# marksho-sfdc/TransmogrifAI

Measured on AMD Instinct MI355X. Metric: end-to-end AutoML wall-clock + hold-out AuPR, 10M-row binary-class tabular, lower is better.
Workload: dtype fp32; 1 GPU; binary-10m; model=BinaryClassificationModelSelector(default grid), rows=10000000, raw_columns=200, cv_folds=3, global_batch=10000000, max_training_sample=1000000, parallelism=single

## Files before the change

transmogrifai_amd/ops/csrc/hip/tree_hist_kernels.hip:

```cpp
#include <hip/hip_runtime.h>
#include <algorithm>
#include <cstdlib>
#include <stdint.h>
#include <math.h>

#include "common/tree_rules.hpp"
#include "hip/tmog_hip_abi.h"
#include "hip/tree_dev.hpp"

namespace {

using namespace tmog;

template <int MODE>
__device__ __forceinline__ int4 stage_row(uint32_t e, int64_t model, int64_t stride, const float* __restrict__ y,
                                          const float* __restrict__ t1, const float* __restrict__ t2,
                                          const float* __restrict__ qs, int wide) {
  const int64_t r = ent_row(e, wide);
  const float w = (float)ent_w(e, wide);
  int4 s;
  s.x = (int)e;
  if (MODE == 0) {
    s.y = (int)ent_w(e, wide); s.z = (int)y[r]; s.w = 0;
  } else if (MODE == 1) {
    const float t = t1[model * stride + r];
    const float wt = w * t;
    s.y = (int)ent_w(e, wide);
    s.z = (int)rintf(wt * qs[1]);
    s.w = (int)rintf((wt * t) * qs[2]);
  } else {
    s.y = (int)rintf((w * t1[model * stride + r]) * qs[0]);
    s.z = (int)rintf((w * t2[model * stride + r]) * qs[1]);
    s.w = 0;
  }
  return s;
}

template <int MODE>
__device__ __forceinline__ void add_row(int* my, int bin, int S, int s0, int Sc, const int4& st) {
  if (MODE == 0) {
    const int c = st.z - s0;
    if (c >= 0 && c < Sc) atomicAdd(my + bin * Sc + c, st.y);
  } else if (MODE == 1) {
    int* hb = my + bin * Sc;
    const int v[3] = {st.y, st.z, st.w};
    for (int k = 0; k < Sc; ++k) atomicAdd(hb + k, v[s0 + k]);
  } else {
    int* hb = my + bin * Sc;
    if (Sc == 2) {
      atomicAdd(hb, st.y); atomicAdd(hb + 1, st.z);
    } else {
      atomicAdd(hb, s0 ? st.z : st.y);
    }
  }
}

constexpr int kCsrU = 16;
constexpr int kCsrG = 8;

template <bool MAX>
__device__ __forceinline__ int wave_reduce32(int v) {
#define TM_DPP_STEP(CTRL, ROWS)                                                         \
  {                                                                                     \
    const int t = __builtin_amdgcn_update_dpp(0, v, CTRL, ROWS, 0xF, false);           \
    v = MAX ? max(v, t) : v + t;                                                        \
  }
  TM_DPP_STEP(0x111, 0xF) TM_DPP_STEP(0x112, 0xF) TM_DPP_STEP(0x114, 0xF) TM_DPP_STEP(0x118, 0xF)
  TM_DPP_STEP(0x142, 0xA) TM_DPP_STEP(0x143, 0xC)
#undef TM_DPP_STEP
  return __builtin_amdgcn_readlane(v, 63);
}

__device__ __forceinline__ void hist_csr_item(const HistItem& it, const uint32_t* __restrict__ rows,
                                              const int32_t* __restrict__ node_model,
                                              const int64_t* __restrict__ node_hist_off, int64_t* __restrict__ hist,
                                              int B, int S, const float* __restrict__ t1,
                                              const float* __restrict__ t2, int64_t stride,
                                              const float* __restrict__ qscale, int skip_bin,
                                              const int64_t* __restrict__ csr_ptr,
                                              const uint16_t* __restrict__ csr_col, int* lds,
                                              const int2* __restrict__ gh, int wide) {
  const int nf = it.nf;
  int* a0 = lds;
  int* a1 = lds + nf;
  const int lane = threadIdx.x & 63;
  const int wave = threadIdx.x >> 6;
  const int nwaves = blockDim.x >> 6;
  const int soff = (2 * nf + 3) & ~3;
  int4* stg = reinterpret_cast<int4*>(lds + soff) + wave * 64;
  int* lens = lds + soff + 4 * 64 * nwaves + wave * 64;
  for (int i = threadIdx.x; i < 2 * nf; i += blockDim.x) lds[i] = 0;
  __syncthreads();
  const int64_t model = node_model ? node_model[it.node] : 0;
  const float* qs = qscale + model * S;
  const uint32_t* rp = rows + it.begin;
  const int64_t cnt = it.count;
  const float* t1m = t1 + model * stride;
  const float* t2m = t2 + model * stride;
  const int64_t step = (int64_t)nwaves * 64;
  const int2* ghp = gh ? gh + it.begin : nullptr;
  uint32_t e_n = 0;
  float g_n = 0.f, h_n = 0.f;
  int2 q_n = make_int2(0, 0);
  int64_t p0_n = 0, p1_n = 0;
  if ((int64_t)wave * 64 < cnt) {
    const int64_t i0 = min((int64_t)wave * 64 + lane, cnt - 1);
    e_n = rp[i0];
    const int64_t r = ent_row(e_n, wide);
    if (ghp) q_n = ghp[i0];
    else { g_n = t1m[r]; h_n = t2m[r]; }
    p0_n = csr_ptr[r]; p1_n = csr_ptr[r + 1];
  }
  for (int64_t base = (int64_t)wave * 64; base < cnt; base += step) {
    const int nrows = (int)min((int64_t)64, cnt - base);
    const float wt = (float)ent_w(e_n, wide);
    int4 mine;
    mine.x = (int)e_n;
    mine.y = ghp ? q_n.x : (int)rintf((wt * g_n) * qs[0]);
    mine.z = ghp ? q_n.y : (int)rintf((wt * h_n) * qs[1]);
    mine.w = 0;
    const int64_t q0 = p0_n;
    const int len = lane < nrows ? (int)(p1_n - p0_n) : 0;
    const bool more = base + step < cnt;
    const int64_t i_n = min(base + step + lane, cnt - 1);
    if (more) e_n = rp[i_n];
    stg[lane] = make_int4(mine.y, mine.z, (int)(uint32_t)(uint64_t)q0, (int)((uint64_t)q0 >> 32));
    lens[lane] = len;
    const int mx = wave_reduce32<true>(len);
    const int W = mx <= 8 ? 8 : mx <= 16 ? 16 : mx <= 32 ? 32 : 64;
    const int RPI = 64 / W;
    const int rs = lane / W, k = lane - rs * W;
    __builtin_amdgcn_s_waitcnt(0xC07F);
    __builtin_amdgcn_wave_barrier();
    for (int j0 = 0; j0 < nrows; j0 += RPI * kCsrG) {
      int col[kCsrG];
      bool ok[kCsrG];
#pragma unroll
      for (int u = 0; u < kCsrG; ++u) {
        const int src = j0 + u * RPI + rs;
        const int sl = min(src, 63);
        const int ln = src < nrows ? lens[sl] : 0;
        const int4 rr = stg[sl];
        const int64_t k0 = (int64_t)(((uint64_t)(uint32_t)rr.w << 32) | (uint64_t)(uint32_t)rr.z);
        ok[u] = k < ln;
        col[u] = csr_col[ok[u] ? k0 + k : k0 > 0 ? k0 - 1 : 0];
      }
      __builtin_amdgcn_sched_barrier(0);
      if (j0 == 0 && more) {
        const int64_t r = ent_row(e_n, wide);
        if (ghp) q_n = ghp[i_n];
        else { g_n = t1m[r]; h_n = t2m[r]; }
        p0_n = csr_ptr[r]; p1_n = csr_ptr[r + 1];
      }
      __builtin_amdgcn_sched_barrier(0);
#pragma unroll
      for (int u = 0; u < kCsrG; ++u)
        if (ok[u]) {
          const int2 gh = *reinterpret_cast<const int2*>(&stg[min(j0 + u * RPI + rs, 63)]);
          atomicAdd(a0 + col[u], gh.x);
          atomicAdd(a1 + col[u], gh.y);
        }
      if (W == 64) {
#pragma unroll
        for (int u = 0; u < kCsrG; ++u) {
          const int src = j0 + u * RPI + rs;
          const int sl = min(src, 63);
          const int ln = src < nrows ? lens[sl] : 0;
          if (ln <= 64) continue;
          const int4 rr = stg[sl];
          const int64_t k0 = (int64_t)(((uint64_t)(uint32_t)rr.w << 32) | (uint64_t)(uint32_t)rr.z);
          for (int kk = k + 64; kk < ln; kk += 64) {
            const int c = csr_col[k0 + kk];
            atomicAdd(a0 + c, rr.x);
            atomicAdd(a1 + c, rr.y);
          }
        }
      }
    }
    __builtin_amdgcn_wave_barrier();
  }
  __syncthreads();
  int64_t* out = hist + node_hist_off[it.node] + (int64_t)it.fg0 * B * S;
  const int per = B * S;
  const bool excl = (it.excl & TMOG_ITEM_SOLE) != 0;
  for (int k = threadIdx.x; k < nf * S; k += blockDim.x) {
    const int f = k / S, s = k - f * S;
    const int v = s ? a1[f] : a0[f];
    int64_t* w = out + (int64_t)f * per + s;
    if (excl) *w = v;
    else if (v != 0) atomicAdd(reinterpret_cast<unsigned long long*>(w), (unsigned long long)(int64_t)v);
  }
}


constexpr int kWideU = 16;

__device__ __forceinline__ void hist_wide_item(const HistItem& it, const uint8_t* __restrict__ Xb, int F, int col0,
                                               const uint32_t* __restrict__ rows,
                                               const int32_t* __restrict__ node_model,
                                               const int64_t* __restrict__ node_hist_off, int64_t* __restrict__ hist,
                                               int B, const float* __restrict__ t1, const float* __restrict__ t2,
                                               int64_t stride, const float* __restrict__ qscale, int skip_bin,
                                               int* lds, const int2* __restrict__ gh, int wide) {
  const int FG = it.nf;
  const int ND = (FG + 3) >> 2;
  const int NP = ND <= 1 ? 1 : ND <= 2 ? 2 : ND <= 4 ? 4 : ND <= 8 ? 8 : 16;
  const int RPI = 64 / NP;
  const int lane = threadIdx.x & 63, wave = threadIdx.x >> 6, nwaves = blockDim.x >> 6;
  const int rs = lane / NP, d = lane - rs * NP;
  const int pos = lane & 15;
  const int sub = (B + 1) * 16;
  unsigned long long* tab = reinterpret_cast<unsigned long long*>(lds);
  const int twords = 4 * sub;
  const int toff = (2 * twords + 3) & ~3;
  int4* stage = reinterpret_cast<int4*>(lds + toff) + wave * 64;
  int* tot = lds + toff + 4 * 64 * nwaves;
  for (int i = threadIdx.x; i < twords; i += blockDim.x) tab[i] = 0ull;
  if (threadIdx.x < 2) tot[threadIdx.x] = 0;
  __syncthreads();
  const bool sparse = skip_bin >= 0;
  const int64_t model = node_model ? node_model[it.node] : 0;
  const float* qs = qscale + model * 2;
  const uint32_t* rp = rows + it.begin;
  const int64_t cnt = it.count;
  const uint64_t xbase = (uint64_t)(uintptr_t)(Xb + col0);
  const uint32_t xlo = __builtin_amdgcn_readfirstlane((uint32_t)xbase);
  const uint32_t xhi = __builtin_amdgcn_readfirstlane((uint32_t)(xbase >> 32));
  const __amdgpu_buffer_rsrc_t xrs = __builtin_amdgcn_make_buffer_rsrc(
      (void*)(uintptr_t)(((uint64_t)xhi << 32) | xlo), (short)0, 0x7FFFFFFF, 0x00020000);
  const uint32_t lane_off = 4u * (uint32_t)min(d, ND - 1);
  const float* t1m = t1 + model * stride;
  const float* t2m = t2 + model * stride;
  const int64_t step = (int64_t)nwaves * 64;
  const int2* ghp = gh ? gh + it.begin : nullptr;
  uint32_t e_n = 0;
  float g_n = 0.f, h_n = 0.f;
  int2 q_n = make_int2(0, 0);
  if ((int64_t)wave * 64 < cnt) {
    const int64_t i0 = min((int64_t)wave * 64 + lane, cnt - 1);
    e_n = rp[i0];
    if (ghp) q_n = ghp[i0];
    else {
      g_n = t1m[ent_row(e_n, wide)];
      h_n = t2m[ent_row(e_n, wide)];
    }
  }
  for (int64_t base = (int64_t)wave * 64; base < cnt; base += step) {
    const int nrows = (int)min((int64_t)64, cnt - base);
    const float wt = (float)ent_w(e_n, wide);
    int4 mine;
    mine.x = (int)e_n;
    mine.y = ghp ? q_n.x : (int)rintf((wt * g_n) * qs[0]);
    mine.z = ghp ? q_n.y : (int)rintf((wt * h_n) * qs[1]);
    mine.w = 0;
    const bool more = base + step < cnt;
    const int64_t i_n = min(base + step + lane, cnt - 1);
    if (more) {
      e_n = rp[i_n];
      if (ghp) q_n = ghp[i_n];
    }
    stage[lane] = make_int4(mine.y, mine.z, mine.x, 0);
    if (sparse) {
      const int a = wave_reduce32<false>(lane < nrows ? mine.y : 0);
      const int b = wave_reduce32<false>(lane < nrows ? mine.z : 0);
      if (lane == 0) {
        atomicAdd(tot, a);
        atomicAdd(tot + 1, b);
      }
    }
    __builtin_amdgcn_s_waitcnt(0xC07F);
    __builtin_amdgcn_wave_barrier();
    {
      uint32_t off[kWideU], w[kWideU];
#pragma unroll
      for (int u = 0; u < kWideU; ++u)
        off[u] = (wide ? (uint32_t)stage[min(u * RPI + rs, 63)].z * (uint32_t)F
                       : __umul24((uint32_t)stage[min(u * RPI + rs, 63)].z & 0xFFFFFFu, (uint32_t)F)) + lane_off;
#pragma unroll
      for (int u = 0; u < kWideU; ++u) w[u] = __builtin_amdgcn_raw_buffer_load_b32(xrs, (int)off[u], 0, 0);
      __builtin_amdgcn_sched_barrier(0);
      if (more && !ghp) {
        g_n = t1m[ent_row(e_n, wide)];
        h_n = t2m[ent_row(e_n, wide)];
      }
      __builtin_amdgcn_sched_barrier(0);
#pragma unroll
      for (int u = 0; u < kWideU; ++u) {
        const bool live = u * RPI + rs < nrows;
        const int2 st = *reinterpret_cast<const int2*>(&stage[min(u * RPI + rs, 63)]);
        const unsigned long long pk = live ? ((unsigned long long)(uint32_t)st.x << 32) + (unsigned long long)(uint32_t)st.y
                                           : 0ull;
#pragma unroll
        for (int k = 0; k < 4; ++k) {
          const int bin = (int)((w[u] >> (8 * k)) & 0xFFu);
          atomicAdd(tab + k * sub + bin * 16 + pos, 4 * d + k < FG ? pk : 0ull);
        }
      }
    }
    __builtin_amdgcn_wave_barrier();
  }
  __syncthreads();
  if (NP < 16) {
    for (int i = threadIdx.x; i < 4 * B * NP; i += blockDim.x) {
      const int r = i / NP, dd = i - r * NP;
      unsigned long long* row = tab + (r / B) * sub + (r % B) * 16;
      unsigned long long acc = row[dd];
      for (int c = NP; c < 16; c += NP) acc += row[c + dd];
      row[dd] = acc;
    }
    __syncthreads();
  }
  auto tix = [sub](int f, int b) { return (f & 3) * sub + b * 16 + (f >> 2); };
  if (sparse) {
    for (int f = threadIdx.x; f < FG; f += blockDim.x) {
      long long g = 0, h = 0;
      for (int b = 0; b < B; ++b) {
        if (b == skip_bin) continue;
        const unsigned long long v = tab[tix(f, b)];
        g += (long long)v >> 32;
        h += (long long)(v & 0xFFFFFFFFull);
      }
      const long long mg = (long long)tot[0] - g, mh = (long long)tot[1] - h;
      tab[tix(f, B)] = ((unsigned long long)mg << 32) + (unsigned long long)(uint32_t)mh;
    }
    __syncthreads();
  }
  int64_t* out = hist + node_hist_off[it.node] + (int64_t)it.fg0 * B * 2;
  const bool excl = (it.excl & TMOG_ITEM_SOLE) != 0;
  for (int k = threadIdx.x; k < FG * B; k += blockDim.x) {
    const int f = k / B, b = k - f * B;
    const unsigned long long v = tab[tix(f, (sparse && b == skip_bin) ? B : b)];
    const int64_t g = (long long)v >> 32, h = (long long)(v & 0xFFFFFFFFull);
    int64_t* o = out + (int64_t)k * 2;
    if (excl) {
      o[0] = g;
      o[1] = h;
    } else {
      if (g != 0) atomicAdd(reinterpret_cast<unsigned long long*>(o), (unsigned long long)g);
      if (h != 0) atomicAdd(reinterpret_cast<unsigned long long*>(o + 1), (unsigned long long)h);
    }
  }
}

constexpr int HIST_U = 16;

__device__ int g_hist_debug = 0;

template <int OCC>
__global__ void __launch_bounds__(256) __attribute__((amdgpu_waves_per_eu(OCC))) hist_wide_kernel(
    const uint8_t* __restrict__ Xb, int F, const uint32_t* __restrict__ rows, const HistItem* __restrict__ items,
    const int32_t* __restrict__ node_feat_off, const int32_t* __restrict__ feat_list,
    const int32_t* __restrict__ node_model, const int64_t* __restrict__ node_hist_off, int64_t* __restrict__ hist,
    int B, const float* __restrict__ t1, const float* __restrict__ t2, int64_t stride,
    const float* __restrict__ qscale, int skip_bin, const int2* __restrict__ gh, int wide,
    const uint8_t* __restrict__ Xh, int Fh) {
  extern __shared__ int lds_w[];
  if (g_hist_debug & 2) return;
  const HistItem it = items[blockIdx.x];
  hist_wide_item(it, Xh, Fh, feat_list[node_feat_off[it.node] + it.fg0], rows, node_model, node_hist_off, hist, B,
                 t1, t2, stride, qscale, skip_bin, lds_w, gh, wide);
}


template <int MODE, bool GEN = true>
__global__ void __launch_bounds__(256) hist_build_kernel(
    const uint8_t* __restrict__ Xb, int F, const uint32_t* __restrict__ rows, const HistItem* __restrict__ items,
    const int32_t* __restrict__ node_feat_off, const int32_t* __restrict__ feat_list,
    const int32_t* __restrict__ node_model, const int64_t* __restrict__ node_hist_off, int64_t* __restrict__ hist,
    int B, int S, const float* __restrict__ y, const float* __restrict__ t1, const float* __restrict__ t2,
    int64_t stride, const float* __restrict__ qscale, int skip_bin, const int64_t* __restrict__ csr_ptr,
    const uint16_t* __restrict__ csr_col, int Sc, const int2* __restrict__ gh, const int* __restrict__ dcount,
    int wide, const uint8_t* __restrict__ Xh, int Fh) {
  extern __shared__ __attribute__((aligned(16))) int lds[];
  if (dcount != nullptr && (int)blockIdx.x >= *dcount) return;
  const HistItem it = items[blockIdx.x];
  const int s0 = ((it.excl >> TMOG_ITEM_SC_SHIFT) & 0xFF) * Sc;
  const int sc = min(Sc, S - s0);
  if (MODE == 2 && g_hist_debug) {
    if ((g_hist_debug & 1) && (it.excl & TMOG_ITEM_CSR)) return;
    if ((g_hist_debug & 2) && !(it.excl & TMOG_ITEM_CSR)) return;
  }
  if (MODE == 2 && (it.excl & TMOG_ITEM_CSR)) {
    hist_csr_item(it, rows, node_model, node_hist_off, hist, B, S, t1, t2, stride, qscale, skip_bin, csr_ptr,
                  csr_col, lds, gh, wide);
    return;
  }
  if (MODE == 2 && (it.excl & TMOG_ITEM_WIDE)) {
    hist_wide_item(it, Xh, Fh, feat_list[node_feat_off[it.node] + it.fg0], rows, node_model, node_hist_off, hist, B,
                   t1, t2, stride, qscale, skip_bin, lds, gh, wide);
    return;
  }
  if constexpr (!GEN) {
    return;
  } else {
  const int FG = it.nf;
  const int R = 64 / FG;
  const int rowstride = B * sc + 1;
  const int ncopy_words = R * FG * rowstride;
  const int lane = threadIdx.x & 63;
  const int wave = threadIdx.x >> 6;
  const int nwaves = blockDim.x >> 6;
  int4* stage = reinterpret_cast<int4*>(lds + ((ncopy_words + 3) & ~3)) + wave * 64;
  int* tot = lds + ((ncopy_words + 3) & ~3) + 4 * 64 * 4;
  const bool sparse = MODE == 2 && skip_bin >= 0;
  const bool regacc = sparse && (it.excl & TMOG_ITEM_REG);
  const bool excl = (it.excl & TMOG_ITEM_SOLE) != 0;
  for (int i = threadIdx.x; i < ncopy_words; i += blockDim.x) lds[i] = 0;
  if (threadIdx.x < TM_MAX_S) tot[threadIdx.x] = 0;
  __syncthreads();

  const int rsub = lane / FG;
  const int fidx = lane - rsub * FG;
  const bool active = rsub < R;
  const int feat = active ? feat_list[node_feat_off[it.node] + it.fg0 + fidx] : 0;
  const int64_t model = node_model ? node_model[it.node] : 0;
  const float* qs = qscale + model * S;
  int* my = lds + (rsub * FG + fidx) * rowstride;
  const uint32_t* rp = rows + it.begin;
  const int64_t cnt = it.count;

  int racc0 = 0, racc1 = 0;
  for (int64_t base = (int64_t)wave * 64; base < cnt; base += (int64_t)nwaves * 64) {
    const int64_t ri = min(base + lane, cnt - 1);
    const int nrows = (int)min((int64_t)64, cnt - base);
    int4 mine;
    if (MODE == 2 && gh) {
      const int2 q = gh[it.begin + ri];
      mine = make_int4((int)rp[ri], q.x, q.y, 0);
    } else {
      mine = stage_row<MODE>(rp[ri], model, stride, y, t1, t2, qs, wide);
    }
    stage[lane] = mine;
    if (sparse) {
      const int a = wave_reduce32<false>(lane < nrows ? mine.y : 0);
      const int b = wave_reduce32<false>(lane < nrows ? mine.z : 0);
      if (lane == 0) {
        atomicAdd(tot, a);
        atomicAdd(tot + 1, b);
      }
    }
    __builtin_amdgcn_s_waitcnt(0xC07F);
    __builtin_amdgcn_wave_barrier();
    if (regacc) {
      for (int j0 = 0; j0 < nrows; j0 += R * 8) {
        int4 st[8];
        int bin[8];
#pragma unroll
        for (int u = 0; u < 8; ++u) st[u] = stage[min(j0 + u * R + rsub, 63)];
#pragma unroll
        for (int u = 0; u < 8; ++u) bin[u] = (int)Xb[(int64_t)ent_row((uint32_t)st[u].x, wide) * F + feat];
#pragma unroll
        for (int u = 0; u < 8; ++u) {
          const bool hit = j0 + u * R + rsub < nrows && bin[u] == 0;
          racc0 += hit ? st[u].y : 0;
          racc1 += hit ? st[u].z : 0;
        }
      }
      __builtin_amdgcn_wave_barrier();
      continue;
    }
    for (int j0 = 0; j0 < nrows; j0 += R * HIST_U) {
      int4 st[HIST_U];
      int bin[HIST_U];
#pragma unroll
      for (int u = 0; u < HIST_U; ++u) st[u] = stage[min(j0 + u * R + rsub, 63)];
#pragma unroll
      for (int u = 0; u < HIST_U; ++u) bin[u] = (int)Xb[(int64_t)ent_row((uint32_t)st[u].x, wide) * F + feat];
#pragma unroll
      for (int u = 0; u < HIST_U; ++u)
        if (active && j0 + u * R + rsub < nrows && bin[u] != skip_bin) add_row<MODE>(my, bin[u], S, s0, sc, st[u]);
    }
    __builtin_amdgcn_wave_barrier();
  }
  __syncthreads();

  int64_t* out = hist + node_hist_off[it.node] + (int64_t)it.fg0 * B * S;
  const int words = FG * B * S;
  if (regacc) {
    if (active) {
      atomicAdd(my, racc0);
      atomicAdd(my + 1, racc1);
    }
    __syncthreads();
  }
  if (sparse) {
    if (R > 1) {
      for (int k = threadIdx.x; k < words; k += blockDim.x) {
        const int f = k / (B * S);
        const int rem = k - f * (B * S);
        int acc = 0;
        for (int r = 0; r < R; ++r) acc += lds[(r * FG + f) * rowstride + rem];
        lds[f * rowstride + rem] = acc;
      }
      __syncthreads();
    }
    for (int t = threadIdx.x; t < FG * S; t += blockDim.x) {
      const int f = t / S, s = t - (t / S) * S;
      int* row = lds + f * rowstride;
      int sum = 0;
      for (int b = 0; b < B; ++b) sum += (b == skip_bin) ? 0 : row[b * S + s];
      row[skip_bin * S + s] = tot[s] - sum;
    }
    __syncthreads();
    const int wlimit = (it.excl & TMOG_ITEM_LIVE0) ? S : B * S;
    for (int k = threadIdx.x; k < words; k += blockDim.x) {
      const int f = k / (B * S);
      if (k - f * (B * S) >= wlimit) continue;
      const int64_t acc = lds[f * rowstride + (k - f * (B * S))];
      if (excl) out[k] = acc;
      else if (acc != 0) atomicAdd(reinterpret_cast<unsigned long long*>(out + k), (unsigned long long)acc);
    }
    return;
  }
  const int cwords = FG * B * sc;
  for (int k = threadIdx.x; k < cwords; k += blockDim.x) {
    const int f = k / (B * sc);
    const int rem = k - f * (B * sc);
    int64_t acc = 0;
    for (int r = 0; r < R; ++r) acc += lds[(r * FG + f) * rowstride + rem];
    const int bin = rem / sc, c = rem - bin * sc;
    int64_t* w = out + ((int64_t)f * B + bin) * S + s0 + c;
    if (excl) *w = acc;
    else if (acc != 0) atomicAdd(reinterpret_cast<unsigned long long*>(w), (unsigned long long)acc);
  }
  }
}

__device__ __forceinline__ int live_word(int k, int dense, int per, int S) {
  if (dense < 0 || k < dense) return k;
  const int t = k - dense, f = t / S;
  return dense + f * per + (t - f * S);
}

__global__ void hist_subtract_kernel(int64_t* __restrict__ hist, const int64_t* __restrict__ parent,
                                     const int64_t* __restrict__ parent_off, const int64_t* __restrict__ small_off,
                                     const int64_t* __restrict__ out_off, const int64_t* __restrict__ size, int n,
                                     int64_t dense, int per, int S) {
  const int j = blockIdx.y;
  if (j >= n) return;
  const int sz = (int)live_words(size[j], dense, per, S);
  const int dn = (int)dense;
  const int64_t* p = parent + parent_off[j];
  const int64_t* s = hist + small_off[j];
  int64_t* o = hist + out_off[j];
  for (int k = blockIdx.x * blockDim.x + threadIdx.x; k < sz; k += gridDim.x * blockDim.x) {
    const int w = live_word(k, dn, per, S);
    o[w] = p[w] - s[w];
  }
}

__global__ void zero_segments_kernel(int64_t* __restrict__ hist, const int64_t* __restrict__ off,
                                     const int64_t* __restrict__ size, int n, int64_t dense, int per, int S,
                                     int n_dense, const int* __restrict__ dcnt) {
  const int j = blockIdx.y;
  if (dcnt != nullptr) {
    n = dcnt[0];
    n_dense = dcnt[1];
  }
  if (j >= n) return;
  int64_t* o = hist + off[j];
  const int64_t dj = j < n_dense ? dense : 0;
  const int sz = (int)live_words(size[j], dj, per, S);
  const int dn = (int)dj;
  for (int k = blockIdx.x * blockDim.x + threadIdx.x; k < sz; k += gridDim.x * blockDim.x)
    o[live_word(k, dn, per, S)] = 0;
}

inline size_t hist_lds_bytes(int B, int Sc) {
  return (size_t)(((64 * (B * Sc + 1)) + 3) & ~3) * sizeof(int) + 4 * 64 * sizeof(int4) + TM_MAX_S * sizeof(int);
}
inline size_t hist_wide_lds_bytes(int B) {
  return (size_t)((2 * (64 * (B + 1) + 17) + 3) & ~3) * sizeof(int) + 4 * 64 * sizeof(int4) + 4 * sizeof(int);
}

}

int tmog::prime_tree_hist() { return prime_kernel(&zero_segments_kernel); }

extern "C" {

int tmog_hip_debug_flags(int flags) {
  return (int)hipMemcpyToSymbol(HIP_SYMBOL(g_hist_debug), &flags, sizeof(int));
}

int tmog_hip_hist_build(const uint8_t* Xb, int F, const uint32_t* rows, const void* items, int n_items,
                        const int32_t* node_feat_off, const int32_t* feat_list, const int32_t* node_model,
                        const int64_t* node_hist_off, int64_t* hist, int B, int mode, int S, const float* y,
                        const float* t1, const float* t2, int64_t stride, const float* qscale, int skip_bin,
                        const int64_t* csr_ptr, const uint16_t* csr_col, int Sc, int n_wide, int need_general,
                        hipStream_t stream, const int32_t* gh_words, const int* dcount, int wide_rows,
                        const uint8_t* Xh, int Fh) {
  if (n_items == 0) return 0;
  if (Xh == nullptr) {
    Xh = Xb;
    Fh = F;
  }
  if (dcount != nullptr && n_wide != 0) return -2;
  const int2* gh = reinterpret_cast<const int2*>(gh_words);
  if (gh && mode != 2) return -2;
  if (Sc <= 0 || Sc > S) Sc = S;
  size_t lds = hist_lds_bytes(B, Sc);
  if (mode == 2 && S == 2) lds = std::max(lds, hist_wide_lds_bytes(B));
  if (lds > 160 * 1024) return -2;
  if (skip_bin >= B || (mode == 2 && skip_bin >= 0 && (S != 2 || Sc != S))) return -2;
  if (mode == 0 && S > TM_WIDE_MAX_S) return -2;
  if ((csr_ptr != nullptr) != (csr_col != nullptr) || (csr_ptr && (mode != 2 || skip_bin <= 0))) return -2;
  const HistItem* it = (const HistItem*)items;
  if (n_wide < 0 || n_wide > n_items || (n_wide > 0 && (mode != 2 || S != 2))) return -2;
  static const bool split_wide = [] { const char* e = std::getenv("TMOG_HIST_WIDE_SPLIT"); return e && e[0] == '1'; }();
  if (!split_wide) n_wide = 0;
  if (n_wide > 0) {
    static const int occ = [] { const char* e = std::getenv("TMOG_HIST_WIDE_OCC"); return e ? std::atoi(e) : 6; }();
#define TM_HIST_WIDE(OCC)                                                                                      \
  hipLaunchKernelGGL(hist_wide_kernel<OCC>, dim3(n_wide), dim3(256), lds, stream, Xb, F, rows, it, node_feat_off, \
                     feat_list, node_model, node_hist_off, hist, B, t1, t2, stride, qscale, skip_bin, gh, wide_rows, Xh, Fh)
    if (occ >= 7) TM_HIST_WIDE(7);
    else TM_HIST_WIDE(6);
#undef TM_HIST_WIDE
    it += n_wide;
    n_items -= n_wide;
    if (n_items == 0) return (int)hipGetLastError();
  }
  const int skip = (mode == 0 || mode == 1) ? -1 : skip_bin;
#define TM_HIST(...)                                                                                           \
  hipLaunchKernelGGL((hist_build_kernel<__VA_ARGS__>), dim3(n_items), dim3(256), lds, stream, Xb, F, rows, it, \
                     node_feat_off, feat_list, node_model, node_hist_off, hist, B, S, y, t1, t2, stride, qscale, \
                     skip, csr_ptr, csr_col, Sc, gh, dcount, wide_rows, Xh, Fh)
  if (mode == 0) TM_HIST(0);
  else if (mode == 1) TM_HIST(1);
  else if (need_general) TM_HIST(2);
  else TM_HIST(2, false);
#undef TM_HIST
  return (int)hipGetLastError();
}

int tmog_hip_hist_subtract(int64_t* hist, const int64_t* parent, const int64_t* parent_off, const int64_t* small_off,
                           const int64_t* out_off, const int64_t* size, int n, int64_t max_size, int64_t dense,
                           int per, int S, hipStream_t stream) {
  if (n == 0) return 0;
  if (max_size >= (int64_t)1 << 31) return -2;
  int gx = (int)min((live_words(max_size, dense, per, S) + 255) / 256, (int64_t)1024);
  if (gx < 1) gx = 1;
  hipLaunchKernelGGL(hist_subtract_kernel, dim3(gx, n), dim3(256), 0, stream, hist, parent, parent_off, small_off,
                     out_off, size, n, dense, per, S);
  return (int)hipGetLastError();
}

int tmog_hip_zero_segments(int64_t* hist, const int64_t* off, const int64_t* size, int n, int64_t max_size,
                           int64_t dense, int per, int S, hipStream_t stream, int n_dense, const int* dn) {
  if (n == 0) return 0;
  if (max_size >= (int64_t)1 << 31) return -2;
  const int64_t lw = std::max(live_words(max_size, dense, per, S), live_words(max_size, 0, per, S));
  int gx = (int)min((lw + 255) / 256, (int64_t)1024);
  if (gx < 1) gx = 1;
  hipLaunchKernelGGL(zero_segments_kernel, dim3(gx, n), dim3(256), 0, stream, hist, off, size, n, dense, per, S,
                     n_dense, dn);
  return (int)hipGetLastError();
}

int tmog_hip_tree_prime() {
  for (int (*prime)() : {prime_tree_hist, prime_tree_split, prime_tree_partition, prime_forest_predict})
    if (const int rc = prime()) return rc;
  return 0;
}

int tmog_hip_hist_stat_chunk(int B, int S) {
  int sc = S;
  while (sc > 1 && hist_lds_bytes(B, sc) > 160 * 1024) --sc;
  return sc;
}

}
```

Measured before the change: 1.566 s per end-to-end AutoML train.

## Replace LDS staging with register/DPP broadcasts in CSR and wide histogram kernels

Adds a LANE variant, on by default, to the CSR and wide histogram bodies. In the CSR body, each row's CSR length is packed into the high bits of the staged offset word, so the separate lens array and its extra LDS read go away, and the gradient pair is kept in registers. In the wide body, when NP is 16, row offsets and gradients are broadcast with DPP row_bcast instead of a store to LDS, a waitcnt and a wave barrier, and the sparse per-wave totals are accumulated in registers with one atomic at the end. It also adds compile-time diagnostic modes and an env var to fall back to LDS staging; packing the length into 16 bits assumes CSR offsets fit in 48 bits and row lengths fit in 16 bits.

```diff
diff --git a/transmogrifai_amd/ops/csrc/hip/tree_hist_kernels.hip b/transmogrifai_amd/ops/csrc/hip/tree_hist_kernels.hip
--- a/transmogrifai_amd/ops/csrc/hip/tree_hist_kernels.hip
+++ b/transmogrifai_amd/ops/csrc/hip/tree_hist_kernels.hip
@@ -55,6 +55,14 @@
   }
 }
 
+#ifndef TMOG_HIST_DIAG
+#define TMOG_HIST_DIAG 0
+#endif
+#if TMOG_HIST_DIAG == 1
+#define TM_LDS_ADD(P, V) (diag_sink += (uint32_t)(uintptr_t)(P) ^ (uint32_t)(V) ^ (uint32_t)((unsigned long long)(V) >> 32))
+#else
+#define TM_LDS_ADD(P, V) atomicAdd(P, V)
+#endif
 constexpr int kCsrU = 16;
 constexpr int kCsrG = 8;
 
@@ -71,6 +79,14 @@
   return __builtin_amdgcn_readlane(v, 63);
 }
 
+template <bool LANE>
+__device__ __forceinline__ void csr_slot(const int4& rr, int len_lds, bool in_chunk, int& ln, int64_t& k0) {
+  const uint32_t hi = (uint32_t)rr.w;
+  ln = in_chunk ? (LANE ? (int)(hi >> 16) : len_lds) : 0;
+  k0 = (int64_t)(((uint64_t)(LANE ? hi & 0xFFFFu : hi) << 32) | (uint64_t)(uint32_t)rr.z);
+}
+
+template <bool LANE>
 __device__ __forceinline__ void hist_csr_item(const HistItem& it, const uint32_t* __restrict__ rows,
                                               const int32_t* __restrict__ node_model,
                                               const int64_t* __restrict__ node_hist_off, int64_t* __restrict__ hist,
@@ -84,7 +100,7 @@
   int* a0 = lds;
   int* a1 = lds + nf;
   const int lane = threadIdx.x & 63;
-  const int wave = threadIdx.x >> 6;
+  const int wave = LANE ? __builtin_amdgcn_readfirstlane(threadIdx.x >> 6) : threadIdx.x >> 6;
   const int nwaves = blockDim.x >> 6;
   const int soff = (2 * nf + 3) & ~3;
   int4* stg = reinterpret_cast<int4*>(lds + soff) + wave * 64;
@@ -99,6 +115,7 @@
   const float* t2m = t2 + model * stride;
   const int64_t step = (int64_t)nwaves * 64;
   const int2* ghp = gh ? gh + it.begin : nullptr;
+  [[maybe_unused]] uint32_t diag_sink = 0;
   uint32_t e_n = 0;
   float g_n = 0.f, h_n = 0.f;
   int2 q_n = make_int2(0, 0);
@@ -109,7 +126,8 @@
     const int64_t r = ent_row(e_n, wide);
     if (ghp) q_n = ghp[i0];
     else { g_n = t1m[r]; h_n = t2m[r]; }
-    p0_n = csr_ptr[r]; p1_n = csr_ptr[r + 1];
+    const int64_t rl = TMOG_HIST_DIAG == 2 ? ent_row(rp[0], wide) : r;
+    p0_n = csr_ptr[rl]; p1_n = csr_ptr[rl + 1];
   }
   for (int64_t base = (int64_t)wave * 64; base < cnt; base += step) {
     const int nrows = (int)min((int64_t)64, cnt - base);
@@ -124,8 +142,13 @@
     const bool more = base + step < cnt;
     const int64_t i_n = min(base + step + lane, cnt - 1);
     if (more) e_n = rp[i_n];
-    stg[lane] = make_int4(mine.y, mine.z, (int)(uint32_t)(uint64_t)q0, (int)((uint64_t)q0 >> 32));
-    lens[lane] = len;
+    if constexpr (LANE) {
+      stg[lane] = make_int4(mine.y, mine.z, (int)(uint32_t)(uint64_t)q0,
+                            (int)((uint32_t)((uint64_t)q0 >> 32) | ((uint32_t)len << 16)));
+    } else {
+      stg[lane] = make_int4(mine.y, mine.z, (int)(uint32_t)(uint64_t)q0, (int)((uint64_t)q0 >> 32));
+      lens[lane] = len;
+    }
     const int mx = wave_reduce32<true>(len);
     const int W = mx <= 8 ? 8 : mx <= 16 ? 16 : mx <= 32 ? 32 : 64;
     const int RPI = 64 / W;
@@ -135,13 +158,16 @@
     for (int j0 = 0; j0 < nrows; j0 += RPI * kCsrG) {
       int col[kCsrG];
       bool ok[kCsrG];
+      [[maybe_unused]] int2 ghk[LANE ? kCsrG : 1];
 #pragma unroll
       for (int u = 0; u < kCsrG; ++u) {
         const int src = j0 + u * RPI + rs;
         const int sl = min(src, 63);
-        const int ln = src < nrows ? lens[sl] : 0;
         const int4 rr = stg[sl];
-        const int64_t k0 = (int64_t)(((uint64_t)(uint32_t)rr.w << 32) | (uint64_t)(uint32_t)rr.z);
+        int ln;
+        int64_t k0;
+        csr_slot<LANE>(rr, LANE ? 0 : lens[sl], src < nrows, ln, k0);
+        if constexpr (LANE) ghk[u] = make_int2(rr.x, rr.y);
         ok[u] = k < ln;
         col[u] = csr_col[ok[u] ? k0 + k : k0 > 0 ? k0 - 1 : 0];
       }
@@ -150,35 +176,45 @@
         const int64_t r = ent_row(e_n, wide);
         if (ghp) q_n = ghp[i_n];
         else { g_n = t1m[r]; h_n = t2m[r]; }
-        p0_n = csr_ptr[r]; p1_n = csr_ptr[r + 1];
+        const int64_t rl = TMOG_HIST_DIAG == 2 ? ent_row(rp[0], wide) : r;
+        p0_n = csr_ptr[rl]; p1_n = csr_ptr[rl + 1];
       }
       __builtin_amdgcn_sched_barrier(0);
 #pragma unroll
       for (int u = 0; u < kCsrG; ++u)
         if (ok[u]) {
-          const int2 gh = *reinterpret_cast<const int2*>(&stg[min(j0 + u * RPI + rs, 63)]);
-          atomicAdd(a0 + col[u], gh.x);
-          atomicAdd(a1 + col[u], gh.y);
+          if constexpr (LANE) {
+            TM_LDS_ADD(a0 + col[u], ghk[u].x);
+            TM_LDS_ADD(a1 + col[u], ghk[u].y);
+          } else {
+            const int2 gh = *reinterpret_cast<const int2*>(&stg[min(j0 + u * RPI + rs, 63)]);
+            TM_LDS_ADD(a0 + col[u], gh.x);
+            TM_LDS_ADD(a1 + col[u], gh.y);
+          }
         }
       if (W == 64) {
 #pragma unroll
         for (int u = 0; u < kCsrG; ++u) {
           const int src = j0 + u * RPI + rs;
           const int sl = min(src, 63);
-          const int ln = src < nrows ? lens[sl] : 0;
+          const int4 rr = stg[sl];
+          int ln;
+          int64_t k0;
+          csr_slot<LANE>(rr, LANE ? 0 : lens[sl], src < nrows, ln, k0);
           if (ln <= 64) continue;
-          const int4 rr = stg[sl];
-          const int64_t k0 = (int64_t)(((uint64_t)(uint32_t)rr.w << 32) | (uint64_t)(uint32_t)rr.z);
           for (int kk = k + 64; kk < ln; kk += 64) {
             const int c = csr_col[k0 + kk];
-            atomicAdd(a0 + c, rr.x);
-            atomicAdd(a1 + c, rr.y);
+            TM_LDS_ADD(a0 + c, rr.x);
+            TM_LDS_ADD(a1 + c, rr.y);
           }
         }
       }
     }
     __builtin_amdgcn_wave_barrier();
   }
+#if TMOG_HIST_DIAG == 1
+  if (diag_sink == 0x9E3779B9u) atomicAdd(lds, 1);
+#endif
   __syncthreads();
   int64_t* out = hist + node_hist_off[it.node] + (int64_t)it.fg0 * B * S;
   const int per = B * S;
@@ -195,6 +231,13 @@
 
 constexpr int kWideU = 16;
 
+template <int U>
+__device__ __forceinline__ int row_bcast(int v) {
+  return __builtin_amdgcn_update_dpp(0, v, 0x150 + U, 0xF, 0xF, false);
+}
+#define TM_ROW16(X) X(0) X(1) X(2) X(3) X(4) X(5) X(6) X(7) X(8) X(9) X(10) X(11) X(12) X(13) X(14) X(15)
+
+template <bool LANE>
 __device__ __forceinline__ void hist_wide_item(const HistItem& it, const uint8_t* __restrict__ Xb, int F, int col0,
                                                const uint32_t* __restrict__ rows,
                                                const int32_t* __restrict__ node_model,
@@ -206,7 +249,8 @@
   const int ND = (FG + 3) >> 2;
   const int NP = ND <= 1 ? 1 : ND <= 2 ? 2 : ND <= 4 ? 4 : ND <= 8 ? 8 : 16;
   const int RPI = 64 / NP;
-  const int lane = threadIdx.x & 63, wave = threadIdx.x >> 6, nwaves = blockDim.x >> 6;
+  const int lane = threadIdx.x & 63, nwaves = blockDim.x >> 6;
+  const int wave = LANE ? __builtin_amdgcn_readfirstlane(threadIdx.x >> 6) : threadIdx.x >> 6;
   const int rs = lane / NP, d = lane - rs * NP;
   const int pos = lane & 15;
   const int sub = (B + 1) * 16;
@@ -245,11 +289,14 @@
       h_n = t2m[ent_row(e_n, wide)];
     }
   }
+  [[maybe_unused]] uint32_t diag_sink = 0;
+  const bool bcast = LANE && NP == 16;
+  int tot_g = 0, tot_h = 0;
   for (int64_t base = (int64_t)wave * 64; base < cnt; base += step) {
     const int nrows = (int)min((int64_t)64, cnt - base);
     const float wt = (float)ent_w(e_n, wide);
     int4 mine;
-    mine.x = (int)e_n;
+    mine.x = TMOG_HIST_DIAG == 2 ? (int)rp[0] : (int)e_n;
     mine.y = ghp ? q_n.x : (int)rintf((wt * g_n) * qs[0]);
     mine.z = ghp ? q_n.y : (int)rintf((wt * h_n) * qs[1]);
     mine.w = 0;
@@ -259,23 +306,24 @@
       e_n = rp[i_n];
       if (ghp) q_n = ghp[i_n];
     }
-    stage[lane] = make_int4(mine.y, mine.z, mine.x, 0);
+    const int qg = lane < nrows ? mine.y : 0, qh = lane < nrows ? mine.z : 0;
     if (sparse) {
-      const int a = wave_reduce32<false>(lane < nrows ? mine.y : 0);
-      const int b = wave_reduce32<false>(lane < nrows ? mine.z : 0);
-      if (lane == 0) {
+      const int a = wave_reduce32<false>(qg);
+      const int b = wave_reduce32<false>(qh);
+      if constexpr (LANE) {
+        tot_g += a;
+        tot_h += b;
+      } else if (lane == 0) {
         atomicAdd(tot, a);
         atomicAdd(tot + 1, b);
       }
     }
-    __builtin_amdgcn_s_waitcnt(0xC07F);
-    __builtin_amdgcn_wave_barrier();
-    {
+    if (bcast) {
+      const uint32_t ro = wide ? mine.x * (uint32_t)F : __umul24((uint32_t)mine.x & 0xFFFFFFu, (uint32_t)F);
       uint32_t off[kWideU], w[kWideU];
-#pragma unroll
-      for (int u = 0; u < kWideU; ++u)
-        off[u] = (wide ? (uint32_t)stage[min(u * RPI + rs, 63)].z * (uint32_t)F
-                       : __umul24((uint32_t)stage[min(u * RPI + rs, 63)].z & 0xFFFFFFu, (uint32_t)F)) + lane_off;
+#define TM_OFF(U) off[U] = (uint32_t)row_bcast<U>((int)ro) + lane_off;
+      TM_ROW16(TM_OFF)
+#undef TM_OFF
 #pragma unroll
       for (int u = 0; u < kWideU; ++u) w[u] = __builtin_amdgcn_raw_buffer_load_b32(xrs, (int)off[u], 0, 0);
       __builtin_amdgcn_sched_barrier(0);
@@ -284,6 +332,36 @@
         h_n = t2m[ent_row(e_n, wide)];
       }
       __builtin_amdgcn_sched_barrier(0);
+#define TM_ADD(U)                                                                                              \
+  {                                                                                                            \
+    const unsigned long long pk = ((unsigned long long)(uint32_t)row_bcast<U>(qg) << 32) +                     \
+                                  (unsigned long long)(uint32_t)row_bcast<U>(qh);                              \
+    _Pragma("unroll") for (int k = 0; k < 4; ++k) {                                                            \
+      const int bin = (int)((w[U] >> (8 * k)) & 0xFFu);                                                        \
+      TM_LDS_ADD(tab + k * sub + bin * 16 + pos, 4 * d + k < FG ? pk : 0ull);                                  \
+    }                                                                                                          \
+  }
+      TM_ROW16(TM_ADD)
+#undef TM_ADD
+      continue;
+    }
+    stage[lane] = make_int4(mine.y, mine.z, mine.x, 0);
+    __builtin_amdgcn_s_waitcnt(0xC07F);
+    __builtin_amdgcn_wave_barrier();
+    {
+      uint32_t off[kWideU], w[kWideU];
+#pragma unroll
+      for (int u = 0; u < kWideU; ++u)
+        off[u] = (wide ? (uint32_t)stage[min(u * RPI + rs, 63)].z * (uint32_t)F
+                       : __umul24((uint32_t)stage[min(u * RPI + rs, 63)].z & 0xFFFFFFu, (uint32_t)F)) + lane_off;
+#pragma unroll
+      for (int u = 0; u < kWideU; ++u) w[u] = __builtin_amdgcn_raw_buffer_load_b32(xrs, (int)off[u], 0, 0);
+      __builtin_amdgcn_sched_barrier(0);
+      if (more && !ghp) {
+        g_n = t1m[ent_row(e_n, wide)];
+        h_n = t2m[ent_row(e_n, wide)];
+      }
+      __builtin_amdgcn_sched_barrier(0);
 #pragma unroll
       for (int u = 0; u < kWideU; ++u) {
         const bool live = u * RPI + rs < nrows;
@@ -293,11 +371,18 @@
 #pragma unroll
         for (int k = 0; k < 4; ++k) {
           const int bin = (int)((w[u] >> (8 * k)) & 0xFFu);
-          atomicAdd(tab + k * sub + bin * 16 + pos, 4 * d + k < FG ? pk : 0ull);
+          TM_LDS_ADD(tab + k * sub + bin * 16 + pos, 4 * d + k < FG ? pk : 0ull);
         }
       }
     }
     __builtin_amdgcn_wave_barrier();
+  }
+#if TMOG_HIST_DIAG == 1
+  if (diag_sink == 0x9E3779B9u) atomicAdd(tot, 1);
+#endif
+  if (LANE && sparse && lane == 0) {
+    atomicAdd(tot, tot_g);
+    atomicAdd(tot + 1, tot_h);
   }
   __syncthreads();
   if (NP < 16) {
@@ -346,7 +431,7 @@
 
 __device__ int g_hist_debug = 0;
 
-template <int OCC>
+template <int OCC, bool LANE>
 __global__ void __launch_bounds__(256) __attribute__((amdgpu_waves_per_eu(OCC))) hist_wide_kernel(
     const uint8_t* __restrict__ Xb, int F, const uint32_t* __restrict__ rows, const HistItem* __restrict__ items,
     const int32_t* __restrict__ node_feat_off, const int32_t* __restrict__ feat_list,
@@ -357,12 +442,12 @@
   extern __shared__ int lds_w[];
   if (g_hist_debug & 2) return;
   const HistItem it = items[blockIdx.x];
-  hist_wide_item(it, Xh, Fh, feat_list[node_feat_off[it.node] + it.fg0], rows, node_model, node_hist_off, hist, B,
-                 t1, t2, stride, qscale, skip_bin, lds_w, gh, wide);
-}
-
-
-template <int MODE, bool GEN = true>
+  hist_wide_item<LANE>(it, Xh, Fh, feat_list[node_feat_off[it.node] + it.fg0], rows, node_model, node_hist_off, hist,
+                       B, t1, t2, stride, qscale, skip_bin, lds_w, gh, wide);
+}
+
+
+template <int MODE, bool GEN = true, bool LANE = true>
 __global__ void __launch_bounds__(256) hist_build_kernel(
     const uint8_t* __restrict__ Xb, int F, const uint32_t* __restrict__ rows, const HistItem* __restrict__ items,
     const int32_t* __restrict__ node_feat_off, const int32_t* __restrict__ feat_list,
@@ -381,13 +466,13 @@
     if ((g_hist_debug & 2) && !(it.excl & TMOG_ITEM_CSR)) return;
   }
   if (MODE == 2 && (it.excl & TMOG_ITEM_CSR)) {
-    hist_csr_item(it, rows, node_model, node_hist_off, hist, B, S, t1, t2, stride, qscale, skip_bin, csr_ptr,
+    hist_csr_item<LANE>(it, rows, node_model, node_hist_off, hist, B, S, t1, t2, stride, qscale, skip_bin, csr_ptr,
                   csr_col, lds, gh, wide);
     return;
   }
   if (MODE == 2 && (it.excl & TMOG_ITEM_WIDE)) {
-    hist_wide_item(it, Xh, Fh, feat_list[node_feat_off[it.node] + it.fg0], rows, node_model, node_hist_off, hist, B,
-                   t1, t2, stride, qscale, skip_bin, lds, gh, wide);
+    hist_wide_item<LANE>(it, Xh, Fh, feat_list[node_feat_off[it.node] + it.fg0], rows, node_model, node_hist_off, hist,
+                         B, t1, t2, stride, qscale, skip_bin, lds, gh, wide);
     return;
   }
   if constexpr (!GEN) {
@@ -573,6 +658,11 @@
   return (size_t)((2 * (64 * (B + 1) + 17) + 3) & ~3) * sizeof(int) + 4 * 64 * sizeof(int4) + 4 * sizeof(int);
 }
 
+bool hist_lane_bodies() {
+  const char* e = std::getenv("TMOG_HIST_LDS_STAGE");
+  return !(e && e[0] == '1');
+}
+
 }
 
 int tmog::prime_tree_hist() { return prime_kernel(&zero_segments_kernel); }
@@ -609,13 +699,16 @@
   if (n_wide < 0 || n_wide > n_items || (n_wide > 0 && (mode != 2 || S != 2))) return -2;
   static const bool split_wide = [] { const char* e = std::getenv("TMOG_HIST_WIDE_SPLIT"); return e && e[0] == '1'; }();
   if (!split_wide) n_wide = 0;
+  const bool lane = hist_lane_bodies();
   if (n_wide > 0) {
     static const int occ = [] { const char* e = std::getenv("TMOG_HIST_WIDE_OCC"); return e ? std::atoi(e) : 6; }();
-#define TM_HIST_WIDE(OCC)                                                                                      \
-  hipLaunchKernelGGL(hist_wide_kernel<OCC>, dim3(n_wide), dim3(256), lds, stream, Xb, F, rows, it, node_feat_off, \
+#define TM_HIST_WIDE(OCC, LANE)                                                                                    \
+  hipLaunchKernelGGL((hist_wide_kernel<OCC, LANE>), dim3(n_wide), dim3(256), lds, stream, Xb, F, rows, it, node_feat_off, \
                      feat_list, node_model, node_hist_off, hist, B, t1, t2, stride, qscale, skip_bin, gh, wide_rows, Xh, Fh)
-    if (occ >= 7) TM_HIST_WIDE(7);
-    else TM_HIST_WIDE(6);
+    if (occ >= 7 && lane) TM_HIST_WIDE(7, true);
+    else if (occ >= 7) TM_HIST_WIDE(7, false);
+    else if (lane) TM_HIST_WIDE(6, true);
+    else TM_HIST_WIDE(6, false);
 #undef TM_HIST_WIDE
     it += n_wide;
     n_items -= n_wide;
@@ -628,8 +721,10 @@
                      skip, csr_ptr, csr_col, Sc, gh, dcount, wide_rows, Xh, Fh)
   if (mode == 0) TM_HIST(0);
   else if (mode == 1) TM_HIST(1);
-  else if (need_general) TM_HIST(2);
-  else TM_HIST(2, false);
+  else if (need_general && lane) TM_HIST(2, true, true);
+  else if (need_general) TM_HIST(2, true, false);
+  else if (lane) TM_HIST(2, false, true);
+  else TM_HIST(2, false, false);
 #undef TM_HIST
   return (int)hipGetLastError();
 }
```

Result: no change. 1.567 s per end-to-end AutoML train (+0.0%).
